# Anonymousijcai2024ttnet/scale_imagenet

Measured on AMD Instinct MI355X. Metric: images/sec ImageNet 224x224, TT-small, MI355X; top-1 exact-match, higher is better.
Workload: dtype u16/u32/u64 packed bits (gate path); f32 as prescaled fp16x2 split operands on the 16-bit MFMA (stem, lin1, lin2); 1 GPU; TT_general_imagenet_v2_small forward, batch=256 224x224 per GPU, bit-packed HIP LUT kernels (BASELINE.json configs[1]); batch_per_gpu=256, global_batch=256, batches_in_flight=2, input=float32 NCHW, normalised (the reference's contract), parallelism=batch shard x1

## Files before the change

scale_imagenet_amd/csrc/head.hip:

```cpp

#include <algorithm>
#include <cmath>
#include <type_traits>

#include "ttnet_common.h"

namespace ttnet {

namespace {

typedef float f32x16 __attribute__((ext_vector_type(16)));

typedef _Float16 f16x8 __attribute__((ext_vector_type(8)));
constexpr int NP = SPLIT_PLANES;

#ifndef TT_LIN1_SKIP
#define TT_LIN1_SKIP 0
#endif
constexpr int kLin1Skip = TT_LIN1_SKIP;

#ifndef TT_LIN1_BM
#define TT_LIN1_BM 128
#endif
#ifndef TT_LIN1_WGS
#define TT_LIN1_WGS 256
#endif
constexpr int G_BM = TT_LIN1_BM, G_BN = 128;
constexpr int G_MT = G_BM / 32, G_NT = G_BN / 32;
constexpr int G_KS = 1;
constexpr int G_CHUNK = 1024;
constexpr int G_STAGE = (G_MT + G_NT) * G_KS * NP * G_CHUNK;
#ifndef TT_LIN1_STAGES
#define TT_LIN1_STAGES 4
#endif
constexpr int G_STAGES = TT_LIN1_STAGES;
#ifndef TT_LIN1_WAVES
#define TT_LIN1_WAVES (TT_LIN1_BM / 32)
#endif
constexpr int G_WAVES = TT_LIN1_WAVES;
constexpr int G_WN = G_WAVES / G_MT, NPW = G_NT / G_WN;
static_assert(G_WAVES % G_MT == 0 && G_NT % G_WN == 0, "waves tile the workgroup's output");
constexpr int G_CHUNKS = (G_MT + G_NT) * G_KS * NP;
#ifndef TT_LIN1_LOADERS
#define TT_LIN1_LOADERS 0
#endif
constexpr int G_LOADERS = TT_LIN1_LOADERS;
constexpr int G_THREADS = 64 * (G_WAVES + G_LOADERS);
constexpr int G_LW = G_LOADERS ? G_LOADERS : G_WAVES;
constexpr int G_LOADS = (G_CHUNKS + G_LW - 1) / G_LW;
constexpr int G_LDS = G_STAGES * G_STAGE + G_CHUNK;

#ifdef TT_LIN1_STAMP
__device__ unsigned long long g_lin1_stamps[512][2];
#endif
template <int AUX_A, int AUX_B>
__global__ __launch_bounds__(G_THREADS) void gemm_f16x2_kernel(const uint8_t *__restrict__ Af, const uint8_t *__restrict__ Bf,
                                                         float *__restrict__ part, int M, int N, int KS, int ks_per,
                                                         int n_tiles, int m_tiles, int splits) {
  extern __shared__ __align__(16) uint8_t lds[];
  const int lane = threadIdx.x & 63, wave = __builtin_amdgcn_readfirstlane(threadIdx.x >> 6);
  const bool loader = G_LOADERS ? wave >= G_WAVES : true, consumer = wave < G_WAVES;
  const int lw = G_LOADERS ? (loader ? wave - G_WAVES : 0) : wave;
  int ntile, mtile, slice;
  {
    const int b = blockIdx.x, groups = m_tiles * splits;
    const int lanes8 = groups < 8 ? groups : 8;
    const int round = b / (lanes8 * n_tiles), rem = b % (lanes8 * n_tiles);
    int grp = round * lanes8 + rem % lanes8;
    ntile = rem / lanes8;
    if (round == groups / lanes8) {
      const int left = groups - round * lanes8;
      grp = round * lanes8 + rem % left;
      ntile = rem / left;
    }
    mtile = grp / splits;
    slice = grp % splits;
  }
  const int mt0 = mtile * G_MT, nt0 = ntile * G_NT;
  const int ks_beg = slice * ks_per, iters = ks_per / G_KS;

  const uint8_t *chunk_src[G_LOADS];
  int chunk_lds[G_LOADS];
#pragma unroll
  for (int jj = 0; jj < G_LOADS; ++jj) {
    const int c = lw + G_LW * jj;
    const bool real = c < G_CHUNKS;
    const bool isA = c < G_MT * G_KS * NP;
    const int cc = real ? (isA ? c : c - G_MT * G_KS * NP) : 0;
    const int pl = cc % NP, kk = (cc / NP) % G_KS, tl = cc / (NP * G_KS);
    chunk_src[jj] = (isA || !real ? Af : Bf) +
                    ((((size_t)((isA || !real ? mt0 : nt0) + tl) * KS + ks_beg + kk) * NP + pl) * 64 + lane) * 16;
    chunk_lds[jj] = real ? c * G_CHUNK : -1;
  }
  auto issue = [&](int it, int buf) {
    static_for<0, G_LOADS>([&](auto jc) {
      constexpr int jj = decltype(jc)::value;
      constexpr bool allA = G_LW * jj + G_LW - 1 < G_MT * G_KS * NP, allB = G_LW * jj >= G_MT * G_KS * NP;
      if constexpr (kLin1Skip & 3) {
        const bool isA = lw + G_LW * jj < G_MT * G_KS * NP;
        if (((kLin1Skip & 1) && isA) || ((kLin1Skip & 2) && !isA)) return;
      }
      const auto src = (const __attribute__((address_space(1))) void *)(chunk_src[jj] + (size_t)it * (G_KS * NP * G_CHUNK));
      const auto dst = (__attribute__((address_space(3))) void *)(lds + (chunk_lds[jj] >= 0 ? buf * G_STAGE + chunk_lds[jj] : G_STAGES * G_STAGE));
      if constexpr (allA) __builtin_amdgcn_global_load_lds(src, dst, 16, 0, AUX_A);
      else if constexpr (allB) __builtin_amdgcn_global_load_lds(src, dst, 16, 0, AUX_B);
      else __builtin_amdgcn_global_load_lds(src, dst, 16, 0, 0);
    });
  };

  constexpr int MPW = 1;
  const int wm = wave % G_MT, wn = wave / G_MT;
  f32x16 acc[MPW][NPW];
#pragma unroll
  for (int i = 0; i < MPW; ++i)
#pragma unroll
    for (int j = 0; j < NPW; ++j)
#pragma unroll
      for (int r = 0; r < 16; ++r) acc[i][j][r] = 0.f;

  static_assert(G_KS == 1 && MPW == 1 && NPW == 4, "the fragment pipeline below is written for one k-step per stage and four N-tiles per wave");
  auto wait_landed = [&](int younger) {
    if (younger >= 5) asm volatile("s_waitcnt vmcnt(%0)" ::"n"(5 * G_LOADS) : "memory");
    else if (younger == 4) asm volatile("s_waitcnt vmcnt(%0)" ::"n"(4 * G_LOADS) : "memory");
    else if (younger == 3) asm volatile("s_waitcnt vmcnt(%0)" ::"n"(3 * G_LOADS) : "memory");
    else if (younger == 2) asm volatile("s_waitcnt vmcnt(%0)" ::"n"(2 * G_LOADS) : "memory");
    else if (younger == 1) asm volatile("s_waitcnt vmcnt(%0)" ::"n"(G_LOADS) : "memory");
    else asm volatile("s_waitcnt vmcnt(0)" ::: "memory");
  };
  static_assert(G_STAGES >= 4 && G_STAGES <= 8 && 5 * G_LOADS < 64, "G_STAGES - 1 stages issued ahead; the barrier of k-step it frees slot (it - 1) % G_STAGES");
#ifdef TT_LIN1_STAMP
  const unsigned long long st_c = __builtin_amdgcn_s_memtime(), st_r = __builtin_amdgcn_s_memrealtime();
#endif
  if (loader) {
    for (int p = 0; p < G_STAGES - 1 && p < iters; ++p) issue(p, p);
    wait_landed(min(G_STAGES - 2, iters - 1));
  }
  __builtin_amdgcn_s_barrier();
  typedef uint32_t u32x4 __attribute__((ext_vector_type(4)));
  u32x4 af[2][NP], bq[NPW][NP];
#define TT_DSRD(dst, addr, off) asm volatile("ds_read_b128 %0, %1 offset:%2" : "=&v"(dst) : "v"(addr), "n"(off))
  const uint32_t lds0 = (uint32_t)(uintptr_t)(__attribute__((address_space(3))) void *)lds + (uint32_t)lane * 16u;
  const uint32_t offA = (uint32_t)(wm * NP) * G_CHUNK, offB = (uint32_t)(G_MT * NP + wn * NPW * NP) * G_CHUNK;
  auto tile = [&](int j, const u32x4 (&a_cur)[NP]) {
    if constexpr (kLin1Skip & 4) {
      acc[0][j][0] += __uint_as_float(a_cur[0][0] ^ bq[j][0][0] ^ bq[j][1][0] ^ a_cur[1][0]);
    } else {
      const f16x8 a0 = __builtin_bit_cast(f16x8, a_cur[0]), a1 = __builtin_bit_cast(f16x8, a_cur[1]);
      const f16x8 b0 = __builtin_bit_cast(f16x8, bq[j][0]), b1 = __builtin_bit_cast(f16x8, bq[j][1]);
      acc[0][j] = __builtin_amdgcn_mfma_f32_32x32x16_f16(a1, b0, acc[0][j], 0, 0, 0);
      acc[0][j] = __builtin_amdgcn_mfma_f32_32x32x16_f16(a0, b1, acc[0][j], 0, 0, 0);
      acc[0][j] = __builtin_amdgcn_mfma_f32_32x32x16_f16(a0, b0, acc[0][j], 0, 0, 0);
    }
    __builtin_amdgcn_sched_barrier(0);
  };
  auto kstep = [&](auto par_c, int it) {
    constexpr int P = decltype(par_c)::value;
    u32x4 (&a_cur)[NP] = af[P];
    u32x4 (&a_nxt)[NP] = af[1 - P];
    const uint32_t sb = lds0 + (uint32_t)(it % G_STAGES) * G_STAGE + offB;
    const uint32_t sn = lds0 + (uint32_t)((it + 1) % G_STAGES) * G_STAGE;
    const uint32_t snb = sn + offB, sna = sn + offA;
    TT_DSRD(bq[2][0], sb, 4 * G_CHUNK);
    TT_DSRD(bq[2][1], sb, 5 * G_CHUNK);
    asm volatile("s_waitcnt lgkmcnt(4)" : "+v"(bq[0][0]), "+v"(bq[0][1]), "+v"(a_cur[0]), "+v"(a_cur[1]));
    tile(0, a_cur);
    TT_DSRD(bq[3][0], sb, 6 * G_CHUNK);
    TT_DSRD(bq[3][1], sb, 7 * G_CHUNK);
    asm volatile("s_waitcnt lgkmcnt(4)" : "+v"(bq[1][0]), "+v"(bq[1][1]));
    tile(1, a_cur);
    TT_DSRD(bq[0][0], snb, 0);
    TT_DSRD(bq[0][1], snb, G_CHUNK);
    TT_DSRD(a_nxt[0], sna, 0);
    TT_DSRD(a_nxt[1], sna, G_CHUNK);
    asm volatile("s_waitcnt lgkmcnt(6)" : "+v"(bq[2][0]), "+v"(bq[2][1]));
    tile(2, a_cur);
    TT_DSRD(bq[1][0], snb, 2 * G_CHUNK);
    TT_DSRD(bq[1][1], snb, 3 * G_CHUNK);
    asm volatile("s_waitcnt lgkmcnt(6)" : "+v"(bq[3][0]), "+v"(bq[3][1]));
    tile(3, a_cur);
  };
  if (consumer) {
    const uint32_t s0 = lds0;
    TT_DSRD(bq[0][0], s0 + offB, 0);
    TT_DSRD(bq[0][1], s0 + offB, G_CHUNK);
    TT_DSRD(af[0][0], s0 + offA, 0);
    TT_DSRD(af[0][1], s0 + offA, G_CHUNK);
    TT_DSRD(bq[1][0], s0 + offB, 2 * G_CHUNK);
    TT_DSRD(bq[1][1], s0 + offB, 3 * G_CHUNK);
  }
  auto step = [&](auto par_c, int it) {
    if (loader) wait_landed(max(0, min(it + G_STAGES - 2, iters - 1) - (it + 1)));
    __builtin_amdgcn_s_barrier();
    if (loader && it + G_STAGES - 1 < iters) issue(it + G_STAGES - 1, (it + G_STAGES - 1) % G_STAGES);
    if (consumer) kstep(par_c, it);
  };
#pragma unroll 1
  for (int it = 0; it < iters; it += 2) {
    step(std::integral_constant<int, 0>{}, it);
    if (it + 1 < iters) step(std::integral_constant<int, 1>{}, it + 1);
  }
  if (consumer)
    asm volatile("s_waitcnt lgkmcnt(0)" : "+v"(bq[0][0]), "+v"(bq[0][1]), "+v"(bq[1][0]), "+v"(bq[1][1]), "+v"(af[0][0]), "+v"(af[0][1]),
                 "+v"(af[1][0]), "+v"(af[1][1]));
#undef TT_DSRD
#ifdef TT_LIN1_STAMP
  if (threadIdx.x == 0 && blockIdx.x < 512) {
    g_lin1_stamps[blockIdx.x][0] = __builtin_amdgcn_s_memtime() - st_c;
    g_lin1_stamps[blockIdx.x][1] = 10ull * (__builtin_amdgcn_s_memrealtime() - st_r);
  }
#endif
  if (!consumer) return;
  float4 *dst = (float4 *)part + (size_t)slice * (m_tiles * G_MT) * (n_tiles * G_NT) * 256;
#pragma unroll
  for (int i = 0; i < MPW; ++i)
#pragma unroll
    for (int j = 0; j < NPW; ++j) {
      float4 *tile = dst + ((size_t)(mt0 + wm + i) * (n_tiles * G_NT) + nt0 + wn * NPW + j) * 256 + lane;
#pragma unroll
      for (int g = 0; g < 4; ++g) {
        if ((kLin1Skip & 8) && g) continue;
        tile[g * 64] = make_float4(acc[i][j][4 * g], acc[i][j][4 * g + 1], acc[i][j][4 * g + 2], acc[i][j][4 * g + 3]);
      }
    }
}

__global__ void split_to_frag_kernel(const float *__restrict__ src, uint16_t *__restrict__ dst, int R, int K, int tiles,
                                     float prescale, int ld, int kvalid) {
  const size_t i = (size_t)blockIdx.x * blockDim.x + threadIdx.x;
  const int KS = K / 16;
  if (i >= (size_t)tiles * KS * 64 * 8) return;
  const int j = i % 8, ln = (i / 8) % 64;
  const size_t tk = i / 512;
  const int ks = tk % KS, tl = tk / KS;
  const int row = tl * 32 + (ln & 31), k = ks * 16 + 8 * (ln >> 5) + j;
  const float v = row < R && k < kvalid ? src[(size_t)row * ld + k] * prescale : 0.f;
  uint16_t h1, h2;
  split_f16x2(v, h1, h2);
  const size_t base = ((size_t)tl * KS + ks) * NP;
  dst[((base + 0) * 64 + ln) * 8 + j] = h1;
  dst[((base + 1) * 64 + ln) * 8 + j] = h2;
}

__global__ void frag_to_ref_kernel(const uint16_t *__restrict__ af, float *__restrict__ out, int n, int G, int PP) {
  const size_t t = (size_t)blockIdx.x * blockDim.x + threadIdx.x;
  const size_t per = (size_t)G * PP * 16;
  if (t >= (size_t)n * per) return;
  const int kk = t % 16, pp = (t / 16) % PP, g = (t / (16 * (size_t)PP)) % G;
  const int img = t / per;
  out[(size_t)img * per + ((size_t)(16 * g + kk)) * PP + pp] = load_feature(af, img, G * PP, g * PP + pp, kk);
}

__global__ void head_mid_kernel(const float4 *__restrict__ part, int splits, const float *__restrict__ scale,
                                const float *__restrict__ shift, uint16_t *__restrict__ mid_frag, int M, int N,
                                int polynomial, uint32_t *range_flag, int mt32, int nt32) {
  const size_t i = (size_t)blockIdx.x * blockDim.x + threadIdx.x;
  const size_t per_slice = (size_t)mt32 * nt32 * 256;
  if (i >= per_slice) return;
  const int lane = i & 63, g = (i >> 6) & 3;
  const int nt = (int)((i >> 8) % nt32), mt = (int)((i >> 8) / nt32);
  const int col = nt * 32 + (lane & 31), row0 = mt * 32 + 8 * g + 4 * (lane >> 5);
  if (col >= N || row0 >= M) return;
  double s[4] = {0.0, 0.0, 0.0, 0.0};
#pragma unroll 8
  for (int z = 0; z < splits; ++z) {
    const float4 v = part[(size_t)z * per_slice + i];
    s[0] += (double)v.x; s[1] += (double)v.y; s[2] += (double)v.z; s[3] += (double)v.w;
  }
  const float sc = scale[col], sh = shift[col];
#pragma unroll
  for (int e = 0; e < 4; ++e) {
    if (row0 + e >= M) break;
    float y = fmaf((float)s[e], sc, sh);
    if (polynomial) {
      const float t = __fadd_rn(0.47f, __fmul_rn(0.50f, y));
      y = __fadd_rn(t, __fmul_rn(0.09f, __fmul_rn(y, y)));
    }
    store_feature(mid_frag, row0 + e, (N + 15) / 16, col >> 4, col & 15, y, range_flag);
  }
}

constexpr int L2_WAVES = 8, L2_STAGES = 4;
__global__ __launch_bounds__(64 * L2_WAVES) void lin2_f16x2_kernel(const uint4 *__restrict__ A, const uint4 *__restrict__ B,
                                                                   const float *__restrict__ bias, float inv,
                                                                   float *__restrict__ out, int M, int N, int KS) {
  __shared__ __align__(16) float red[L2_WAVES * 16 * 64];
  const int lane = threadIdx.x & 63, wave = threadIdx.x >> 6;
  const int mt = blockIdx.y, nt = blockIdx.x;
  f32x16 acc;
#pragma unroll
  for (int r = 0; r < 16; ++r) acc[r] = 0.f;
  const int nk = wave < KS ? (KS - wave + L2_WAVES - 1) / L2_WAVES : 0;
  uint4 fa[L2_STAGES][NP], fb[L2_STAGES][NP];
  auto load = [&](int i, uint4 (&a)[NP], uint4 (&b)[NP]) {
    const int ks = wave + L2_WAVES * i;
#pragma unroll
    for (int pl = 0; pl < NP; ++pl) {
      a[pl] = A[(((size_t)mt * KS + ks) * NP + pl) * 64 + lane];
      b[pl] = B[(((size_t)nt * KS + ks) * NP + pl) * 64 + lane];
    }
  };
  static_for<0, L2_STAGES>([&](auto ss) {
    constexpr int sl = decltype(ss)::value;
    if (sl < nk) load(sl, fa[sl], fb[sl]);
  });
  for (int i0 = 0; i0 < nk; i0 += L2_STAGES) {
    static_for<0, L2_STAGES>([&](auto ss) {
      constexpr int sl = decltype(ss)::value;
      if (i0 + sl < nk) {
        const f16x8 a0 = __builtin_bit_cast(f16x8, fa[sl][0]), a1 = __builtin_bit_cast(f16x8, fa[sl][1]);
        const f16x8 b0 = __builtin_bit_cast(f16x8, fb[sl][0]), b1 = __builtin_bit_cast(f16x8, fb[sl][1]);
        acc = __builtin_amdgcn_mfma_f32_32x32x16_f16(a1, b0, acc, 0, 0, 0);
        acc = __builtin_amdgcn_mfma_f32_32x32x16_f16(a0, b1, acc, 0, 0, 0);
        acc = __builtin_amdgcn_mfma_f32_32x32x16_f16(a0, b0, acc, 0, 0, 0);
        if (i0 + sl + L2_STAGES < nk) load(i0 + sl + L2_STAGES, fa[sl], fb[sl]);
      }
    });
  }
#pragma unroll
  for (int r = 0; r < 16; ++r) red[(wave * 16 + r) * 64 + lane] = acc[r];
  __syncthreads();
  for (int e = threadIdx.x; e < 16 * 64; e += 64 * L2_WAVES) {
    double sum = 0.0;
#pragma unroll
    for (int w = 0; w < L2_WAVES; ++w) sum += (double)red[w * (16 * 64) + e];
    const int ln = e & 63, r = e >> 6;
    const int row = mt * 32 + (r & 3) + 8 * (r >> 2) + 4 * (ln >> 5);
    const int col = nt * 32 + (ln & 31);
    if (row < M && col < N) out[(size_t)row * N + col] = (float)(sum * (double)inv + (double)bias[col]);
  }
}

__global__ void permute_lin1_kernel(const float *__restrict__ w1, float *__restrict__ w1p, int O, int G, int PP) {
  const size_t i = (size_t)blockIdx.x * blockDim.x + threadIdx.x;
  const size_t K = (size_t)G * PP * 16;
  if (i >= (size_t)O * K) return;
  const size_t o = i / K, f = i % K;
  const int k = f % 16, pp = (f / 16) % PP, g = f / (16 * (size_t)PP);
  w1p[i] = w1[o * K + ((size_t)(16 * g + k)) * PP + pp];
}

}

int gemm_f16x2_splits(int M, int N, int KS) {
  const int tiles = ((M + G_BM - 1) / G_BM) * ((N + G_BN - 1) / G_BN);
  const int want = std::max(TT_LIN1_WGS / std::max(1, tiles), 8);
  for (int s = std::min(std::min(want, KS / 8), 128); s > 1; --s)
    if (KS % s == 0) return s;
  return 1;
}

size_t gemm_f16x2_part_elems(int M, int N, int KS) {
  const size_t mt = (M + G_BM - 1) / G_BM, nt = (N + G_BN - 1) / G_BN;
  return (size_t)gemm_f16x2_splits(M, N, KS) * mt * G_BM * nt * G_BN;
}

int launch_gemm_f16x2(const void *Af, const void *Bf, float *part, int M, int N, int K, int splits, hipStream_t s) {
  const int KS = K / 16;
  if (K % 16 || KS % splits || (KS / splits) % G_KS) {
    set_error("gemm_f16x2: K=%d not divisible into %d slices of %d k-steps", K, splits, G_KS);
    return TTNET_E_UNSUPPORTED;
  }
  static const int nt = getenv("TTNET_LIN1_NT") ? atoi(getenv("TTNET_LIN1_NT")) : 0;
  const int n_tiles = (N + G_BN - 1) / G_BN, m_tiles = (M + G_BM - 1) / G_BM;
  auto launch = [&](auto kernel) -> int {
    TT_TRY(ensure_dynamic_lds((const void *)kernel, G_LDS));
    hipLaunchKernelGGL(kernel, dim3(n_tiles * m_tiles * splits), dim3(G_THREADS), G_LDS, s, (const uint8_t *)Af, (const uint8_t *)Bf, part, M, N,
                       KS, KS / splits, n_tiles, m_tiles, splits);
    return TTNET_OK;
  };
  if (nt == 11) TT_TRY(launch(gemm_f16x2_kernel<2, 2>));
  else if (nt == 1) TT_TRY(launch(gemm_f16x2_kernel<0, 2>));
  else if (nt == 10) TT_TRY(launch(gemm_f16x2_kernel<2, 0>));
  else TT_TRY(launch(gemm_f16x2_kernel<0, 0>));
  TT_HIP(hipGetLastError());
  return TTNET_OK;
}

size_t frag_elems(int rows, int K) { return (size_t)((rows + 31) / 32) * (K / 16) * NP * 64 * 8; }

float weight_prescale(const float *w, size_t n) {
  float amax = 0.f;
  for (size_t i = 0; i < n; ++i) amax = fmaxf(amax, fabsf(w[i]));
  if (!(amax > 0.f) || !std::isfinite(amax)) return 1.0f;
  int e;
  frexpf(amax, &e);
  int k = 14 - e;
  k = k > 60 ? 60 : (k < -60 ? -60 : k);
  return ldexpf(1.0f, k);
}

int launch_split_to_frag(const float *src, void *dst, int R, int K, int rows_padded, float prescale, hipStream_t s, int ld,
                         int kvalid) {
  if (K % 16) {
    set_error("split_to_frag: K=%d is not a multiple of 16", K);
    return TTNET_E_UNSUPPORTED;
  }
  const int tiles = (rows_padded + 31) / 32;
  const size_t t = (size_t)tiles * (K / 16) * 64 * 8;
  hipLaunchKernelGGL(split_to_frag_kernel, dim3((unsigned)((t + 255) / 256)), dim3(256), 0, s, src, (uint16_t *)dst, R, K, tiles,
                     prescale, ld > 0 ? ld : K, kvalid > 0 ? kvalid : K);
  TT_HIP(hipGetLastError());
  return TTNET_OK;
}

int launch_frag_to_reference_order(const void *af, float *out, int n, int G, int PP, hipStream_t s) {
  const size_t t = (size_t)n * G * PP * 16;
  hipLaunchKernelGGL(frag_to_ref_kernel, dim3((unsigned)((t + 255) / 256)), dim3(256), 0, s, (const uint16_t *)af, out, n, G, PP);
  TT_HIP(hipGetLastError());
  return TTNET_OK;
}

int launch_head_mid(const float *part, int splits, const float *scale, const float *shift, void *mid_frag, int M, int N,
                    int polynomial, uint32_t *range_flag, hipStream_t s) {
  const int mt32 = (M + G_BM - 1) / G_BM * G_MT, nt32 = (N + G_BN - 1) / G_BN * G_NT;
  const size_t t = (size_t)mt32 * nt32 * 256;
  hipLaunchKernelGGL(head_mid_kernel, dim3((unsigned)((t + 255) / 256)), dim3(256), 0, s, (const float4 *)part, splits, scale, shift,
                     (uint16_t *)mid_frag, M, N, polynomial, range_flag, mt32, nt32);
  TT_HIP(hipGetLastError());
  return TTNET_OK;
}

int launch_lin2_f16x2(const void *mid_frag, const void *w2f, const float *bias, float inv, float *out, int M, int N, int K,
                      hipStream_t s) {
  const int KS = (K + 15) / 16;
  hipLaunchKernelGGL(lin2_f16x2_kernel, dim3((N + 31) / 32, (M + 31) / 32), dim3(64 * L2_WAVES), 0, s,
                     (const uint4 *)mid_frag, (const uint4 *)w2f, bias, inv, out, M, N, KS);
  TT_HIP(hipGetLastError());
  return TTNET_OK;
}

int launch_permute_lin1(const float *w1, float *w1p, int O, int G, int PP, hipStream_t s) {
  const size_t t = (size_t)O * G * PP * 16;
  hipLaunchKernelGGL(permute_lin1_kernel, dim3((unsigned)((t + 255) / 256)), dim3(256), 0, s, w1, w1p, O, G, PP);
  TT_HIP(hipGetLastError());
  return TTNET_OK;
}

}
```

Before: 2.133 million images/s.

## Load lin1 A fragments straight to registers, stage only B through LDS

The lin1 split-fp16 GEMM now has each wave load its own A row-tile fragments directly into a register ring of G_STAGES slots via global_load_dwordx4, instead of staging them through LDS. Only B goes through LDS. The k-loop is unrolled by the stage count so slot indices and LDS offsets become compile-time immediates, and the optional loader-wave and configurable BM/waves paths are dropped. This is meant to cut LDS traffic, ds_read count and address arithmetic per k-step. In exchange it uses more VGPRs for the A ring, makes the loop body larger, and hard-codes the tile shape.

```diff
diff --git a/scale_imagenet_amd/csrc/head.hip b/scale_imagenet_amd/csrc/head.hip
--- a/scale_imagenet_amd/csrc/head.hip
+++ b/scale_imagenet_amd/csrc/head.hip
@@ -19,36 +19,21 @@
 #endif
 constexpr int kLin1Skip = TT_LIN1_SKIP;
 
-#ifndef TT_LIN1_BM
-#define TT_LIN1_BM 128
-#endif
 #ifndef TT_LIN1_WGS
 #define TT_LIN1_WGS 256
 #endif
-constexpr int G_BM = TT_LIN1_BM, G_BN = 128;
+constexpr int G_BM = 128, G_BN = 128;
 constexpr int G_MT = G_BM / 32, G_NT = G_BN / 32;
-constexpr int G_KS = 1;
 constexpr int G_CHUNK = 1024;
-constexpr int G_STAGE = (G_MT + G_NT) * G_KS * NP * G_CHUNK;
+constexpr int G_WAVES = G_MT, NPW = G_NT;
+constexpr int G_THREADS = 64 * G_WAVES;
+constexpr int G_STAGE = G_NT * NP * G_CHUNK;
 #ifndef TT_LIN1_STAGES
 #define TT_LIN1_STAGES 4
 #endif
 constexpr int G_STAGES = TT_LIN1_STAGES;
-#ifndef TT_LIN1_WAVES
-#define TT_LIN1_WAVES (TT_LIN1_BM / 32)
-#endif
-constexpr int G_WAVES = TT_LIN1_WAVES;
-constexpr int G_WN = G_WAVES / G_MT, NPW = G_NT / G_WN;
-static_assert(G_WAVES % G_MT == 0 && G_NT % G_WN == 0, "waves tile the workgroup's output");
-constexpr int G_CHUNKS = (G_MT + G_NT) * G_KS * NP;
-#ifndef TT_LIN1_LOADERS
-#define TT_LIN1_LOADERS 0
-#endif
-constexpr int G_LOADERS = TT_LIN1_LOADERS;
-constexpr int G_THREADS = 64 * (G_WAVES + G_LOADERS);
-constexpr int G_LW = G_LOADERS ? G_LOADERS : G_WAVES;
-constexpr int G_LOADS = (G_CHUNKS + G_LW - 1) / G_LW;
-constexpr int G_LDS = G_STAGES * G_STAGE + G_CHUNK;
+constexpr int G_LOADS = ((kLin1Skip & 1) ? 0 : NP) + ((kLin1Skip & 2) ? 0 : NP);
+constexpr int G_LDS = G_STAGES * G_STAGE;
 
 #ifdef TT_LIN1_STAMP
 __device__ unsigned long long g_lin1_stamps[512][2];
@@ -59,8 +44,6 @@
                                                          int n_tiles, int m_tiles, int splits) {
   extern __shared__ __align__(16) uint8_t lds[];
   const int lane = threadIdx.x & 63, wave = __builtin_amdgcn_readfirstlane(threadIdx.x >> 6);
-  const bool loader = G_LOADERS ? wave >= G_WAVES : true, consumer = wave < G_WAVES;
-  const int lw = G_LOADERS ? (loader ? wave - G_WAVES : 0) : wave;
   int ntile, mtile, slice;
   {
     const int b = blockIdx.x, groups = m_tiles * splits;
@@ -77,131 +60,118 @@
     slice = grp % splits;
   }
   const int mt0 = mtile * G_MT, nt0 = ntile * G_NT;
-  const int ks_beg = slice * ks_per, iters = ks_per / G_KS;
-
-  const uint8_t *chunk_src[G_LOADS];
-  int chunk_lds[G_LOADS];
-#pragma unroll
-  for (int jj = 0; jj < G_LOADS; ++jj) {
-    const int c = lw + G_LW * jj;
-    const bool real = c < G_CHUNKS;
-    const bool isA = c < G_MT * G_KS * NP;
-    const int cc = real ? (isA ? c : c - G_MT * G_KS * NP) : 0;
-    const int pl = cc % NP, kk = (cc / NP) % G_KS, tl = cc / (NP * G_KS);
-    chunk_src[jj] = (isA || !real ? Af : Bf) +
-                    ((((size_t)((isA || !real ? mt0 : nt0) + tl) * KS + ks_beg + kk) * NP + pl) * 64 + lane) * 16;
-    chunk_lds[jj] = real ? c * G_CHUNK : -1;
-  }
-  auto issue = [&](int it, int buf) {
-    static_for<0, G_LOADS>([&](auto jc) {
-      constexpr int jj = decltype(jc)::value;
-      constexpr bool allA = G_LW * jj + G_LW - 1 < G_MT * G_KS * NP, allB = G_LW * jj >= G_MT * G_KS * NP;
-      if constexpr (kLin1Skip & 3) {
-        const bool isA = lw + G_LW * jj < G_MT * G_KS * NP;
-        if (((kLin1Skip & 1) && isA) || ((kLin1Skip & 2) && !isA)) return;
+  const int ks_beg = slice * ks_per, iters = ks_per;
+
+  const int wm = wave;
+  const uint8_t *a_src = Af + ((((size_t)(mt0 + wm) * KS + ks_beg) * NP) * 64 + lane) * 16;
+  const uint8_t *b_src = Bf + ((((size_t)(nt0 + wave) * KS + ks_beg) * NP) * 64 + lane) * 16;
+  typedef uint32_t u32x4 __attribute__((ext_vector_type(4)));
+  u32x4 ar[G_STAGES][NP], bq[NPW][NP];
+  if constexpr (kLin1Skip & 1)
+    static_for<0, G_STAGES>([&](auto sc) { ar[decltype(sc)::value][0] = ar[decltype(sc)::value][1] = u32x4{0x3c003c00u, 0x3c003c00u, 0x3c003c00u, 0x3c003c00u}; });
+  auto issue = [&](auto slot_c, int it) {
+    constexpr int SL = decltype(slot_c)::value;
+    if constexpr (!(kLin1Skip & 1)) {
+      const uint8_t *src = a_src + (size_t)it * (NP * G_CHUNK);
+      if constexpr (AUX_A == 2) {
+        asm volatile("global_load_dwordx4 %0, %1, off nt" : "=v"(ar[SL][0]) : "v"(src));
+        asm volatile("global_load_dwordx4 %0, %1, off offset:1024 nt" : "=v"(ar[SL][1]) : "v"(src));
+      } else {
+        asm volatile("global_load_dwordx4 %0, %1, off" : "=v"(ar[SL][0]) : "v"(src));
+        asm volatile("global_load_dwordx4 %0, %1, off offset:1024" : "=v"(ar[SL][1]) : "v"(src));
       }
-      const auto src = (const __attribute__((address_space(1))) void *)(chunk_src[jj] + (size_t)it * (G_KS * NP * G_CHUNK));
-      const auto dst = (__attribute__((address_space(3))) void *)(lds + (chunk_lds[jj] >= 0 ? buf * G_STAGE + chunk_lds[jj] : G_STAGES * G_STAGE));
-      if constexpr (allA) __builtin_amdgcn_global_load_lds(src, dst, 16, 0, AUX_A);
-      else if constexpr (allB) __builtin_amdgcn_global_load_lds(src, dst, 16, 0, AUX_B);
-      else __builtin_amdgcn_global_load_lds(src, dst, 16, 0, 0);
-    });
-  };
-
-  constexpr int MPW = 1;
-  const int wm = wave % G_MT, wn = wave / G_MT;
-  f32x16 acc[MPW][NPW];
-#pragma unroll
-  for (int i = 0; i < MPW; ++i)
-#pragma unroll
-    for (int j = 0; j < NPW; ++j)
-#pragma unroll
-      for (int r = 0; r < 16; ++r) acc[i][j][r] = 0.f;
-
-  static_assert(G_KS == 1 && MPW == 1 && NPW == 4, "the fragment pipeline below is written for one k-step per stage and four N-tiles per wave");
+    }
+    if constexpr (!(kLin1Skip & 2)) {
+      static_for<0, NP>([&](auto pc) {
+        constexpr int PL = decltype(pc)::value;
+        const auto src = (const __attribute__((address_space(1))) void *)(b_src + (size_t)it * (NP * G_CHUNK) + PL * G_CHUNK);
+        const auto dst = (__attribute__((address_space(3))) void *)(lds + SL * G_STAGE + (wave * NP + PL) * G_CHUNK);
+        __builtin_amdgcn_global_load_lds(src, dst, 16, 0, AUX_B);
+      });
+    }
+  };
+  static_assert(G_CHUNK == 1024, "plane 1 of A is addressed by the immediate offset of its load");
+
+  f32x16 acc[NPW];
+#pragma unroll
+  for (int j = 0; j < NPW; ++j)
+#pragma unroll
+    for (int r = 0; r < 16; ++r) acc[j][r] = 0.f;
+
+  static_assert(NPW == 4, "the fragment pipeline below is written for four N-tiles per wave");
   auto wait_landed = [&](int younger) {
-    if (younger >= 5) asm volatile("s_waitcnt vmcnt(%0)" ::"n"(5 * G_LOADS) : "memory");
+    if (younger >= 6) asm volatile("s_waitcnt vmcnt(%0)" ::"n"(6 * G_LOADS) : "memory");
+    else if (younger == 5) asm volatile("s_waitcnt vmcnt(%0)" ::"n"(5 * G_LOADS) : "memory");
     else if (younger == 4) asm volatile("s_waitcnt vmcnt(%0)" ::"n"(4 * G_LOADS) : "memory");
     else if (younger == 3) asm volatile("s_waitcnt vmcnt(%0)" ::"n"(3 * G_LOADS) : "memory");
     else if (younger == 2) asm volatile("s_waitcnt vmcnt(%0)" ::"n"(2 * G_LOADS) : "memory");
     else if (younger == 1) asm volatile("s_waitcnt vmcnt(%0)" ::"n"(G_LOADS) : "memory");
     else asm volatile("s_waitcnt vmcnt(0)" ::: "memory");
   };
-  static_assert(G_STAGES >= 4 && G_STAGES <= 8 && 5 * G_LOADS < 64, "G_STAGES - 1 stages issued ahead; the barrier of k-step it frees slot (it - 1) % G_STAGES");
+  static_assert(G_STAGES >= 4 && G_STAGES <= 8 && 6 * G_LOADS < 64, "G_STAGES - 1 stages issued ahead; the barrier of k-step it frees slot (it - 1) % G_STAGES");
+  static_assert((G_STAGES - 1) * G_STAGE + (2 * NPW - 1) * G_CHUNK < 65536, "fragment reads address a stage by their immediate offset");
 #ifdef TT_LIN1_STAMP
   const unsigned long long st_c = __builtin_amdgcn_s_memtime(), st_r = __builtin_amdgcn_s_memrealtime();
 #endif
-  if (loader) {
-    for (int p = 0; p < G_STAGES - 1 && p < iters; ++p) issue(p, p);
-    wait_landed(min(G_STAGES - 2, iters - 1));
-  }
+  static_for<0, G_STAGES - 1>([&](auto pc) {
+    if (decltype(pc)::value < iters) issue(pc, decltype(pc)::value);
+  });
+  wait_landed(min(G_STAGES - 2, iters - 1));
   __builtin_amdgcn_s_barrier();
-  typedef uint32_t u32x4 __attribute__((ext_vector_type(4)));
-  u32x4 af[2][NP], bq[NPW][NP];
 #define TT_DSRD(dst, addr, off) asm volatile("ds_read_b128 %0, %1 offset:%2" : "=&v"(dst) : "v"(addr), "n"(off))
   const uint32_t lds0 = (uint32_t)(uintptr_t)(__attribute__((address_space(3))) void *)lds + (uint32_t)lane * 16u;
-  const uint32_t offA = (uint32_t)(wm * NP) * G_CHUNK, offB = (uint32_t)(G_MT * NP + wn * NPW * NP) * G_CHUNK;
   auto tile = [&](int j, const u32x4 (&a_cur)[NP]) {
     if constexpr (kLin1Skip & 4) {
-      acc[0][j][0] += __uint_as_float(a_cur[0][0] ^ bq[j][0][0] ^ bq[j][1][0] ^ a_cur[1][0]);
+      acc[j][0] += __uint_as_float(a_cur[0][0] ^ bq[j][0][0] ^ bq[j][1][0] ^ a_cur[1][0]);
     } else {
       const f16x8 a0 = __builtin_bit_cast(f16x8, a_cur[0]), a1 = __builtin_bit_cast(f16x8, a_cur[1]);
       const f16x8 b0 = __builtin_bit_cast(f16x8, bq[j][0]), b1 = __builtin_bit_cast(f16x8, bq[j][1]);
-      acc[0][j] = __builtin_amdgcn_mfma_f32_32x32x16_f16(a1, b0, acc[0][j], 0, 0, 0);
-      acc[0][j] = __builtin_amdgcn_mfma_f32_32x32x16_f16(a0, b1, acc[0][j], 0, 0, 0);
-      acc[0][j] = __builtin_amdgcn_mfma_f32_32x32x16_f16(a0, b0, acc[0][j], 0, 0, 0);
+      acc[j] = __builtin_amdgcn_mfma_f32_32x32x16_f16(a1, b0, acc[j], 0, 0, 0);
+      acc[j] = __builtin_amdgcn_mfma_f32_32x32x16_f16(a0, b1, acc[j], 0, 0, 0);
+      acc[j] = __builtin_amdgcn_mfma_f32_32x32x16_f16(a0, b0, acc[j], 0, 0, 0);
     }
     __builtin_amdgcn_sched_barrier(0);
   };
-  auto kstep = [&](auto par_c, int it) {
-    constexpr int P = decltype(par_c)::value;
-    u32x4 (&a_cur)[NP] = af[P];
-    u32x4 (&a_nxt)[NP] = af[1 - P];
-    const uint32_t sb = lds0 + (uint32_t)(it % G_STAGES) * G_STAGE + offB;
-    const uint32_t sn = lds0 + (uint32_t)((it + 1) % G_STAGES) * G_STAGE;
-    const uint32_t snb = sn + offB, sna = sn + offA;
-    TT_DSRD(bq[2][0], sb, 4 * G_CHUNK);
-    TT_DSRD(bq[2][1], sb, 5 * G_CHUNK);
+  auto kstep = [&](auto slot_c) {
+    constexpr int P = decltype(slot_c)::value;
+    u32x4 (&a_cur)[NP] = ar[P];
+    constexpr int sb = P * G_STAGE, sn = (P + 1) % G_STAGES * G_STAGE;
+    TT_DSRD(bq[2][0], lds0, sb + 4 * G_CHUNK);
+    TT_DSRD(bq[2][1], lds0, sb + 5 * G_CHUNK);
     asm volatile("s_waitcnt lgkmcnt(4)" : "+v"(bq[0][0]), "+v"(bq[0][1]), "+v"(a_cur[0]), "+v"(a_cur[1]));
     tile(0, a_cur);
-    TT_DSRD(bq[3][0], sb, 6 * G_CHUNK);
-    TT_DSRD(bq[3][1], sb, 7 * G_CHUNK);
+    TT_DSRD(bq[3][0], lds0, sb + 6 * G_CHUNK);
+    TT_DSRD(bq[3][1], lds0, sb + 7 * G_CHUNK);
     asm volatile("s_waitcnt lgkmcnt(4)" : "+v"(bq[1][0]), "+v"(bq[1][1]));
     tile(1, a_cur);
-    TT_DSRD(bq[0][0], snb, 0);
-    TT_DSRD(bq[0][1], snb, G_CHUNK);
-    TT_DSRD(a_nxt[0], sna, 0);
-    TT_DSRD(a_nxt[1], sna, G_CHUNK);
-    asm volatile("s_waitcnt lgkmcnt(6)" : "+v"(bq[2][0]), "+v"(bq[2][1]));
+    TT_DSRD(bq[0][0], lds0, sn);
+    TT_DSRD(bq[0][1], lds0, sn + G_CHUNK);
+    asm volatile("s_waitcnt lgkmcnt(4)" : "+v"(bq[2][0]), "+v"(bq[2][1]));
     tile(2, a_cur);
-    TT_DSRD(bq[1][0], snb, 2 * G_CHUNK);
-    TT_DSRD(bq[1][1], snb, 3 * G_CHUNK);
-    asm volatile("s_waitcnt lgkmcnt(6)" : "+v"(bq[3][0]), "+v"(bq[3][1]));
+    TT_DSRD(bq[1][0], lds0, sn + 2 * G_CHUNK);
+    TT_DSRD(bq[1][1], lds0, sn + 3 * G_CHUNK);
+    asm volatile("s_waitcnt lgkmcnt(4)" : "+v"(bq[3][0]), "+v"(bq[3][1]));
     tile(3, a_cur);
   };
-  if (consumer) {
-    const uint32_t s0 = lds0;
-    TT_DSRD(bq[0][0], s0 + offB, 0);
-    TT_DSRD(bq[0][1], s0 + offB, G_CHUNK);
-    TT_DSRD(af[0][0], s0 + offA, 0);
-    TT_DSRD(af[0][1], s0 + offA, G_CHUNK);
-    TT_DSRD(bq[1][0], s0 + offB, 2 * G_CHUNK);
-    TT_DSRD(bq[1][1], s0 + offB, 3 * G_CHUNK);
-  }
-  auto step = [&](auto par_c, int it) {
-    if (loader) wait_landed(max(0, min(it + G_STAGES - 2, iters - 1) - (it + 1)));
+  TT_DSRD(bq[0][0], lds0, 0);
+  TT_DSRD(bq[0][1], lds0, G_CHUNK);
+  TT_DSRD(bq[1][0], lds0, 2 * G_CHUNK);
+  TT_DSRD(bq[1][1], lds0, 3 * G_CHUNK);
+  auto step = [&](auto slot_c, int it) {
+    constexpr int P = decltype(slot_c)::value;
+    if (it + G_STAGES - 2 < iters) asm volatile("s_waitcnt vmcnt(%0)" ::"n"((G_STAGES - 3) * G_LOADS) : "memory");
+    else wait_landed(max(0, iters - 2 - it));
     __builtin_amdgcn_s_barrier();
-    if (loader && it + G_STAGES - 1 < iters) issue(it + G_STAGES - 1, (it + G_STAGES - 1) % G_STAGES);
-    if (consumer) kstep(par_c, it);
+    if (it + G_STAGES - 1 < iters) issue(std::integral_constant<int, (P + G_STAGES - 1) % G_STAGES>{}, it + G_STAGES - 1);
+    kstep(slot_c);
   };
 #pragma unroll 1
-  for (int it = 0; it < iters; it += 2) {
-    step(std::integral_constant<int, 0>{}, it);
-    if (it + 1 < iters) step(std::integral_constant<int, 1>{}, it + 1);
-  }
-  if (consumer)
-    asm volatile("s_waitcnt lgkmcnt(0)" : "+v"(bq[0][0]), "+v"(bq[0][1]), "+v"(bq[1][0]), "+v"(bq[1][1]), "+v"(af[0][0]), "+v"(af[0][1]),
-                 "+v"(af[1][0]), "+v"(af[1][1]));
+  for (int it = 0; it < iters; it += G_STAGES) {
+    static_for<0, G_STAGES>([&](auto pc) {
+      if (decltype(pc)::value == 0 || it + decltype(pc)::value < iters) step(pc, it + decltype(pc)::value);
+    });
+  }
+  asm volatile("s_waitcnt lgkmcnt(0)" : "+v"(bq[0][0]), "+v"(bq[0][1]), "+v"(bq[1][0]), "+v"(bq[1][1]));
 #undef TT_DSRD
 #ifdef TT_LIN1_STAMP
   if (threadIdx.x == 0 && blockIdx.x < 512) {
@@ -209,19 +179,16 @@
     g_lin1_stamps[blockIdx.x][1] = 10ull * (__builtin_amdgcn_s_memrealtime() - st_r);
   }
 #endif
-  if (!consumer) return;
   float4 *dst = (float4 *)part + (size_t)slice * (m_tiles * G_MT) * (n_tiles * G_NT) * 256;
 #pragma unroll
-  for (int i = 0; i < MPW; ++i)
-#pragma unroll
-    for (int j = 0; j < NPW; ++j) {
-      float4 *tile = dst + ((size_t)(mt0 + wm + i) * (n_tiles * G_NT) + nt0 + wn * NPW + j) * 256 + lane;
-#pragma unroll
-      for (int g = 0; g < 4; ++g) {
-        if ((kLin1Skip & 8) && g) continue;
-        tile[g * 64] = make_float4(acc[i][j][4 * g], acc[i][j][4 * g + 1], acc[i][j][4 * g + 2], acc[i][j][4 * g + 3]);
-      }
-    }
+  for (int j = 0; j < NPW; ++j) {
+    float4 *tile = dst + ((size_t)(mt0 + wm) * (n_tiles * G_NT) + nt0 + j) * 256 + lane;
+#pragma unroll
+    for (int g = 0; g < 4; ++g) {
+      if ((kLin1Skip & 8) && g) continue;
+      tile[g * 64] = make_float4(acc[j][4 * g], acc[j][4 * g + 1], acc[j][4 * g + 2], acc[j][4 * g + 3]);
+    }
+  }
 }
 
 __global__ void split_to_frag_kernel(const float *__restrict__ src, uint16_t *__restrict__ dst, int R, int K, int tiles,
@@ -356,8 +323,8 @@
 
 int launch_gemm_f16x2(const void *Af, const void *Bf, float *part, int M, int N, int K, int splits, hipStream_t s) {
   const int KS = K / 16;
-  if (K % 16 || KS % splits || (KS / splits) % G_KS) {
-    set_error("gemm_f16x2: K=%d not divisible into %d slices of %d k-steps", K, splits, G_KS);
+  if (K % 16 || KS % splits) {
+    set_error("gemm_f16x2: K=%d not divisible into %d slices of whole k-steps", K, splits);
     return TTNET_E_UNSUPPORTED;
   }
   static const int nt = getenv("TTNET_LIN1_NT") ? atoi(getenv("TTNET_LIN1_NT")) : 0;
```

Result: slower. 2.087 million images/s (-2.2%).
